# ponder-lab/RoaringBitmap

Hardware: AMD Instinct MI355X
Metric: input GB/s (HBM roofline %) for batched and/or/xor + wide-OR, 1/2/4/8 GPU (higher is better)
Workload: dtype u64

## Files before the change

### roaringbitmap_amd/csrc/pairwise.hip

```cpp
#include <algorithm>
#include "kernels.hpp"
#include "wave.hpp"

namespace rbg {

constexpr int kPairThreads = 256;

#ifndef RBG_SMALL_STUDY
#define RBG_SMALL_STUDY 0
#endif
#if RBG_SMALL_STUDY
constexpr int kStudyWords = 32;
__device__ uint64_t g_small_study[8192 * kStudyWords];
__device__ uint64_t g_merge_ts[8192 * 4][8];
#define RBG_MT(i) if (lane == 0) g_merge_ts[min(blockIdx.x, 8191u) * 4 + (threadIdx.x >> 6)][i] = __builtin_amdgcn_s_memrealtime()
#else
#define RBG_MT(i)
#endif

__device__ __forceinline__ bool keeps_a_only(int op) { return op != RB_AND; }
__device__ __forceinline__ bool keeps_b_only(int op) { return op == RB_OR || op == RB_XOR || is_lazy_op(op); }

__device__ __forceinline__ uint64_t alg_bytes(int t, uint32_t c, uint32_t r) {
  return t == kBitmap ? 8192ull : t == kArray ? 2ull * c : 4ull * r + 2;
// ... 855 lines not shown
  RecU cur = load_rec(recs + g);
  Task tc = decode_task<OP, ROLE == kRoleLight>(cur, pay_a, pay_b);
  uint4 pq[8], qq[8];
#if RBG_STUDY
  uint64_t lt_acc[8] = {0, 0, 0, 0, 0, 0, 0, 0}, lt0 = 0, lt1 = 0, lt2 = 0;
  uint64_t lt_wait = 0;
#define RBG_LT(x) if (ROLE == kRoleLight) { x; }
#define RBG_HT(x) if (ROLE == kRoleHeavy) { x; }
#else
#define RBG_LT(x)
#define RBG_HT(x)
#endif
  if (tc.kind == kCopy || tc.bigq) load_chunks(qq, tc.pp, 16, lane);
  else load_chunks(qq, tc.pq, tc.qbytes, lane);
  load_chunks(pq, tc.pp, tc.bigp ? 16u : tc.pbytes, lane);
  while (true) {
    uint64_t gn = g + stride;
    if (queue) {
      gn = g + 1;
      if (gn >= cend) {
        const Chunk c1 = claim_take(queue, n, qk, qtried, ticket, lane);
        gn = c1.s;
        cend = c1.e;
        if (qtried < kQueueStripes) ticket = claim_issue(queue, qk, lane);
      }
    }
    const bool has_next = gn < n;
    RBG_LT(lt0 = __builtin_amdgcn_s_memtime());
    RBG_HT(lt0 = __builtin_amdgcn_s_memtime());
    const RecU nx = load_rec(recs + (has_next ? gn : g));
    const Task tn = decode_task<OP, ROLE == kRoleLight>(nx, pay_a, pay_b);
    RBG_LT(lt1 = __builtin_amdgcn_s_memtime(); lt_acc[0] += lt1 - lt0);
    RBG_HT(lt1 = __builtin_amdgcn_s_memtime(); lt_acc[0] += lt1 - lt0);
    int ty = kEmpty, c = 0;
    uint32_t nr = 0, cw = 0xFFFFFFFFu;
    uint8_t *dst = out + cur.out;
    bool done = false;
    if (ROLE == kRoleHeavy && OP == RB_AND && tc.tp == kRun && tc.tq == kRun && !tc.bigp &&
        !tc.bigq && ((tc.rp + 3) & ~3u) + tc.rq <= 2048u) {
      int r = 0;
      done = and_runs_intervals<CARD_ONLY>(pq, qq, tc.rp, tc.rq, s, dst, lane, c, r);
      if (done) {
        ty = c == 0 ? kEmpty : CARD_ONLY ? kArray : kRun;
        nr = ty == kRun ? (uint32_t)r : 0u;
        __builtin_amdgcn_sched_barrier(0);
        {
          const bool real = has_next && !tn.bigq;
          load_chunks(qq, real ? tn.pq : tn.pp, real ? tn.qbytes : 16u, lane);
        }
        load_chunks(pq, tn.pp, tn.bigp ? 16u : tn.pbytes, lane);
      }
    }
    if (ROLE == kRoleHeavy && RBG_HEAVY_MERGE && !done && (OP == RB_OR || OP == RB_XOR) && !tm.lazy &&
        tc.tp == kArray && tc.tq == kArray && tc.cp + tc.cq <= kMergeMax) {
      merge_stage(pq, tc.cp, qq, tc.cq, s, lane);
      __builtin_amdgcn_sched_barrier(0);
      {
        const bool real = has_next && !tn.bigq;
        load_chunks(qq, real ? tn.pq : tn.pp, real ? tn.qbytes : 16u, lane);
      }
      load_chunks(pq, tn.pp, tn.bigp ? 16u : tn.pbytes, lane);
      c = (int)merge_run<OP, !CARD_ONLY>(s, tc.cp, tc.cq, reinterpret_cast<uint16_t *>(dst), lane);
      ty = CARD_ONLY ? (c ? kArray : kEmpty) : (c || (OP == RB_XOR && tm.keep_empty)) ? kArray : kEmpty;
      nr = 0;
      done = true;
    }
    if (ROLE == kRoleHeavy && !done) {
#if RBG_STUDY
      {
        const uint64_t tw0 = __builtin_amdgcn_s_memtime();
        __builtin_amdgcn_s_waitcnt(0x0F70);
        lt_wait += __builtin_amdgcn_s_memtime() - tw0;
      }
#endif
      uint64_t w[kW];
      if (bitmap_payload(tc.tp, tc.cp)) {
#pragma unroll
        for (int k = 0; k < 8; ++k) {
          w[2 * k] = pack2(pq[k].x, pq[k].y);
          w[2 * k + 1] = pack2(pq[k].z, pq[k].w);
        }
      } else if (tc.tp == kRun && !tc.bigp) {
        stage_run_toggles(pq, tc.rp, s, lane);
        lds_read_words(s, w, lane);
        wave_lds_sync();
        toggles_to_words(w, lane);
      } else {
        if (tc.bigp) stage_big_runs(tc.pp, tc.rp, s, lane);
        else stage_from_chunks(tc.tp, pq, tc.cp, tc.rp, s, lane);
        lds_read_words(s, w, lane);
        wave_lds_sync();
      }
      if (bitmap_payload(tc.tq, tc.cq)) {
#pragma unroll
        for (int k = 0; k < 8; ++k) {
          word_op<OP>(w[2 * k], pack2(qq[k].x, qq[k].y));
          word_op<OP>(w[2 * k + 1], pack2(qq[k].z, qq[k].w));
        }
      } else if (tc.tq == kRun && !tc.bigq) {
        stage_run_toggles(qq, tc.rq, s, lane);
        uint64_t t[kW];
        lds_read_words(s, t, lane);
        wave_lds_sync();
        toggles_to_words(t, lane);
#pragma unroll
        for (int j = 0; j < kW; ++j) word_op<OP>(w[j], t[j]);
      } else {
        if (tc.bigq) stage_big_runs(tc.pq, tc.rq, s, lane);
        else stage_from_chunks(tc.tq, qq, tc.cq, tc.rq, s, lane);
        const uint4 *s4 = reinterpret_cast<const uint4 *>(s);
#pragma unroll
        for (int k = 0; k < 8; ++k) {
          const uint4 v = s4[k * 64 + lane];
          word_op<OP>(w[2 * k], pack2(v.x, v.y));
          word_op<OP>(w[2 * k + 1], pack2(v.z, v.w));
        }
        wave_lds_sync();
      }
      RBG_HT(lt2 = __builtin_amdgcn_s_memtime(); lt_acc[1] += lt2 - lt1);
      __builtin_amdgcn_sched_barrier(0);
      {
        const bool real = has_next && !tn.bigq;
        load_chunks(qq, real ? tn.pq : tn.pp, real ? tn.qbytes : 16u, lane);
      }
      load_chunks(pq, tn.pp, tn.bigp ? 16u : tn.pbytes, lane);
      const int ta = tc.tp, tb = tc.tq;
      const bool lazy = OP == RB_OR && tm.lazy;
      const bool eff = eff_rule<OP>(ta, tb, tc.cp, tc.cq);
      int r;
      metrics(w, lane, (eff || (lazy && (ta == kRun || tb == kRun))) && !CARD_ONLY, c, r);
      RBG_HT(const uint64_t lt3 = __builtin_amdgcn_s_memtime(); lt_acc[2] += lt3 - lt2; lt2 = lt3);
      bool bits = false;
      if (lazy) {
        ty = lazy_or_type(tm.lazy, ta, tb, tc.cp, tc.cq, c, r, cw, bits);
        if (ty == kRun && c == kSpan) r = 1;
      } else if (OP != RB_OR && c == 0 && !(OP == RB_XOR && tm.keep_empty)) ty = kEmpty;
      else if (eff) ty = type_eff(c, r);
      else if (OP == RB_OR && tm.inplace && ta == kBitmap && tb == kArray) {
        ty = kBitmap;
      } else if (OP == RB_OR && (ta == kBitmap || tb == kBitmap)) {
        ty = type_lr(c);
        if (ty == kRun) r = 1;
      } else ty = type_ab(c);
      if (CARD_ONLY) ty = c ? kArray : kEmpty;
      else if (ty != kEmpty) {
        if (RBG_BAL_EMIT) emit_container_bal(bits ? (int)kBitmap : ty, w, c, r, dst, s, estage[wv], lane);
        else emit_container(bits ? (int)kBitmap : ty, w, c, r, dst, s, lane);
      }
      nr = ty == kRun ? (uint32_t)r : 0u;
      RBG_HT(lt_acc[3 + (ty == kBitmap ? 0 : ty == kArray ? 1 : 2)] += __builtin_amdgcn_s_memtime() - lt2);
    } else if (ROLE != kRoleHeavy) {
      if (tc.kind == kFilter || tc.kind == kBits) {
        if (tc.bigq) stage_big_runs(tc.pq, tc.rq, s, fresh(lane));
        else stage_from_chunks(tc.tq, qq, tc.cq, tc.rq, s, fresh(lane));
      } else if (!CARD_ONLY) {
        if (tc.bigp) {
          copy_payload(tc.pp, dst, tc.pbytes, fresh(lane), qq);
          __builtin_amdgcn_s_waitcnt(0x0F70);
        } else store_chunks(pq, dst, tc.pbytes, fresh(lane));
      }
      {
        const bool real = has_next && tn.kind != kCopy && !tn.bigq;
        load_chunks(qq, real ? tn.pq : tn.pp, real ? tn.qbytes : 16u, fresh(lane));
      }
      RBG_LT(lt2 = __builtin_amdgcn_s_memtime(); lt_acc[tc.kind == kFilter ? 1 + (tc.tq == kBitmap ? 0 : tc.tq == kArray ? 1 : 2) : 4] += lt2 - lt1);
      if (tc.kind == kFilter) {
        uint16_t *o = CARD_ONLY ? nullptr : reinterpret_cast<uint16_t *>(dst);
        uint4 *tb = tbuf[ROLE == kRoleLight ? wv : 0];
        c = OP == RB_ANDNOT ? filter_rows_linear<true, !CARD_ONLY>(pq, (int)tc.cp, s, ob, tb, o, fresh(lane))
                            : filter_rows_linear<false, !CARD_ONLY>(pq, (int)tc.cp, s, ob, tb, o, fresh(lane));
        ty = c ? kArray : kEmpty;
      } else if (tc.kind == kBits) {
        const uint4 *s4 = reinterpret_cast<const uint4 *>(s);
        uint32_t cl = 0;
#pragma unroll
        for (int k = 0; k < 8; ++k) {
          const uint4 x = s4[k * 64 + lane];
          pq[k] = make_uint4(pq[k].x | x.x, pq[k].y | x.y, pq[k].z | x.z, pq[k].w | x.w);
          cl += __popc(pq[k].x) + __popc(pq[k].y) + __popc(pq[k].z) + __popc(pq[k].w);
        }
        c = (int)wave_sum_u32(cl);
        const bool keep_bitmap = tm.inplace && tc.p_is_a && tc.tq == kArray;
        ty = c == kSpan && !keep_bitmap ? kRun : kBitmap;
        nr = ty == kRun ? 1u : 0u;
        if (!CARD_ONLY) {
          uint4 *o4 = reinterpret_cast<uint4 *>(dst);
          if (ty == kRun) {
            if (lane == 0) o4[0] = make_uint4(0xFFFF0000u, 0u, 0u, 0u);
          } else {
#pragma unroll
            for (int k = 0; k < 8; ++k) o4[k * 64 + lane] = pq[k];
          }
        }
        if (CARD_ONLY) {
          ty = kArray;
          nr = 0;
        }
      } else {
        ty = tc.tp;
        c = (int)tc.cp;
        nr = tc.rp;
      }
      RBG_LT(lt_acc[5] += __builtin_amdgcn_s_memtime() - lt2);
      load_chunks(pq, tn.pp, tn.bigp ? 16u : tn.pbytes, fresh(lane));
    }
    wave_lds_sync();
    if (lane == 0) {
      tm.type[cur.t] = (uint8_t)ty;
      tm.res[cur.t] = task_res((uint32_t)ty, nr, cw != 0xFFFFFFFFu ? cw : (uint32_t)c);
    }
    RBG_LT(lt_acc[6] += __builtin_amdgcn_s_memtime() - lt0; ++lt_acc[7]);
    RBG_HT(lt_acc[6] += __builtin_amdgcn_s_memtime() - lt0; ++lt_acc[7]);
    if (!has_next) break;
    g = gn;
    cur = nx;
    tc = tn;
  }
#if RBG_STUDY
  if (ROLE == kRoleLight && lane == 0 && wv == 0 && blockIdx.x % 97 == 0)
    printf("light timing blk %u: decode %lu stageB %lu stageA %lu stageR %lu copy %lu filter %lu iter %lu tasks %lu\n",
           blockIdx.x, lt_acc[0], lt_acc[1], lt_acc[2], lt_acc[3], lt_acc[4], lt_acc[5], lt_acc[6], lt_acc[7]);
  if (ROLE == kRoleHeavy && lane == 0 && wv == 0 && blockIdx.x % 61 == 0)
    printf("heavy timing op %d blk %u: decode %lu build %lu (payload wait %lu) metrics %lu emitB %lu emitA %lu emitR %lu iter %lu tasks %lu\n",
           OP, blockIdx.x, lt_acc[0], lt_acc[1], lt_wait, lt_acc[2], lt_acc[3], lt_acc[4], lt_acc[5], lt_acc[6], lt_acc[7]);
#endif
}

__device__ __forceinline__ uint32_t fold_chunks(const uint4 (&q)[8]) {
  uint32_t x = 0;
#pragma unroll
  for (int i = 0; i < 8; ++i) x ^= q[i].x ^ q[i].y ^ q[i].z ^ q[i].w;
  return x;
}
template <int OP>
__global__ __launch_bounds__(256, 4) void k_probe_tasks(const uint8_t *__restrict__ pay_a,
                                                     const uint8_t *__restrict__ pay_b,
                                                     const TaskRec *__restrict__ recs, uint64_t n, uint32_t *sink) {
  const int lane = lane_id();
  const int wv = __builtin_amdgcn_readfirstlane(threadIdx.x >> 6);
  const uint64_t stride = (uint64_t)gridDim.x * 4;
  uint64_t g = (uint64_t)blockIdx.x * 4 + wv;
  if (g >= n) return;
  RecU cur = load_rec(recs + g);
  Task tc = decode_task<OP, false>(cur, pay_a, pay_b);
  uint4 pq[8], qq[8];
  load_chunks(pq, tc.pp, tc.bigp ? 16u : tc.pbytes, lane);
  if (tc.kind == kCopy || tc.bigq) load_chunks(qq, tc.pp, 16, lane);
  else load_chunks(qq, tc.pq, tc.qbytes, lane);
  uint32_t acc = 0;
  while (true) {
    const uint64_t gn = g + stride;
    const bool has_next = gn < n;
    const RecU nx = load_rec(recs + (has_next ? gn : g));
    const Task tn = decode_task<OP, false>(nx, pay_a, pay_b);
    acc ^= fold_chunks(qq);
    {
      const bool real = has_next && tn.kind != kCopy && !tn.bigq;
      load_chunks(qq, real ? tn.pq : tn.pp, real ? tn.qbytes : 16u, lane);
    }
    acc ^= fold_chunks(pq);
    load_chunks(pq, tn.pp, tn.bigp ? 16u : tn.pbytes, lane);
    if (!has_next) break;
    g = gn;
    tc = tn;
  }
  sink[(uint64_t)blockIdx.x * 256 + threadIdx.x] = acc;
}
__global__ __launch_bounds__(256, 4) void k_probe_stream(const uint8_t *__restrict__ p, uint64_t bytes,
                                                      uint32_t *sink) {
  const int lane = lane_id();
  const uint64_t w = (uint64_t)blockIdx.x * 4 + (threadIdx.x >> 6), nw = (uint64_t)gridDim.x * 4;
  const uint64_t chunks = bytes / 8192;
  uint32_t acc = 0;
  for (uint64_t c = w; c < chunks; c += nw) {
    uint4 q[8];
    load_chunks(q, p + c * 8192, 8192, lane);
    acc ^= fold_chunks(q);
  }
  sink[(uint64_t)blockIdx.x * 256 + threadIdx.x] = acc;
}
void launch_probe(int op, int mode, const uint8_t *pa, const uint8_t *pb, uint64_t a_bytes, const TaskRec *recs,
                  uint64_t n, uint32_t *sink, unsigned blocks, hipStream_t st) {
  if (mode == 2) {
    k_probe_stream<<<blocks, 256, 0, st>>>(pa, a_bytes, sink);
    return;
  }
  if (!n) return;
  switch (op) {
  case RB_AND: k_probe_tasks<RB_AND><<<blocks, 256, 0, st>>>(pa, pb, recs, n, sink); break;
  case RB_OR: k_probe_tasks<RB_OR><<<blocks, 256, 0, st>>>(pa, pb, recs, n, sink); break;
  case RB_XOR: k_probe_tasks<RB_XOR><<<blocks, 256, 0, st>>>(pa, pb, recs, n, sink); break;
  default: k_probe_tasks<RB_ANDNOT><<<blocks, 256, 0, st>>>(pa, pb, recs, n, sink); break;
  }
}

__global__ __launch_bounds__(kPairThreads) void k_compact_count(const uint64_t *tb, uint64_t nseg,
                                                                const uint8_t *ttype, uint64_t *bk) {
  const uint64_t p = (uint64_t)blockIdx.x * kPairThreads + threadIdx.x;
  uint64_t n = 0;
  if (p < nseg)
    for (uint64_t t = tb[p]; t < tb[p + 1]; ++t) n += ttype[t] != kEmpty;
  const uint64_t v[1] = {n};
  uint64_t sum[1];
  block_sums(v, sum);
  if (threadIdx.x == 0) bk[blockIdx.x] = sum[0];
}
__global__ __launch_bounds__(kPairThreads) void k_compact_write(const uint64_t *tb, uint64_t nseg, TaskMeta tm,
                                                                const uint64_t *bks, OutView out,
                                                                const uint32_t *seg_pair, uint64_t *pair_card,
                                                                uint64_t *stats, uint64_t *rseg, uint64_t *rbegin,
                                                                CallTail tail) {
  __shared__ uint32_t wtot[kPairThreads / 64];
  const uint64_t b0 = (uint64_t)blockIdx.x * kPairThreads, be = min(b0 + kPairThreads, nseg);
  const uint64_t p = b0 + threadIdx.x;
  const uint64_t R0 = bks[blockIdx.x];
  uint32_t kept = 0;
  const uint64_t t0 = p < nseg ? tb[p] : 0, t1 = p < nseg ? tb[p + 1] : 0;
  for (uint64_t t = t0; t < t1; ++t) kept += tm.type[t] != kEmpty;
  uint32_t btot;
  const uint64_t rs = R0 + block_xscan(kept, wtot, btot);
  if (p < nseg) {
    if (rseg) rseg[p] = rs;
    if (rbegin) rbegin[p] = rs;
// ... 752 lines not shown
```

### roaringbitmap_amd/csrc/wave.hpp

```cpp
#pragma once
#include "common.hpp"

namespace rbg {

constexpr int kW = 16;

__device__ __forceinline__ void wave_lds_sync() {
  __builtin_amdgcn_fence(__ATOMIC_RELEASE, "wavefront");
  __builtin_amdgcn_wave_barrier();
  __builtin_amdgcn_fence(__ATOMIC_ACQUIRE, "wavefront");
}

__device__ __forceinline__ int lane_id() { return (int)(threadIdx.x & 63); }
__device__ __forceinline__ int fresh(int x) {
  asm volatile("" : "+v"(x));
  return x;
}

__device__ __forceinline__ uint32_t xcd_swizzle(uint32_t orig, uint32_t nwg) {
  const uint32_t q = nwg / 8, r = nwg % 8, xcd = orig % 8;
  return (xcd < r ? xcd * (q + 1) : r * (q + 1) + (xcd - r) * q) + orig / 8;
}

template <int CTRL, int ROW_MASK = 0xf, bool BOUND_ZERO = true>
__device__ __forceinline__ uint32_t dpp(uint32_t x) {
  return (uint32_t)__builtin_amdgcn_update_dpp(0, (int)x, CTRL, ROW_MASK, 0xf, BOUND_ZERO);
}
__device__ __forceinline__ uint32_t readlane(uint32_t x, int l) {
  return (uint32_t)__builtin_amdgcn_readlane((int)x, l);
}
__device__ __forceinline__ uint32_t wave_scan_u32(uint32_t v, int ) {
  v += dpp<0x111>(v);
  v += dpp<0x112>(v);
  v += dpp<0x114>(v);
  v += dpp<0x118>(v);
  v += dpp<0x142, 0xa, false>(v);
  v += dpp<0x143, 0xc, false>(v);
  return v;
}
__device__ __forceinline__ uint32_t wave_xscan_xor(uint32_t v, int ) {
  v ^= dpp<0x111>(v);
  v ^= dpp<0x112>(v);
  v ^= dpp<0x114>(v);
  v ^= dpp<0x118>(v);
  v ^= dpp<0x142, 0xa, false>(v);
  v ^= dpp<0x143, 0xc, false>(v);
  return v;
}
__device__ __forceinline__ uint64_t wave_scan_u64(uint64_t v, int lane) {
  return (uint64_t)wave_scan_u32((uint32_t)v, lane) | ((uint64_t)wave_scan_u32((uint32_t)(v >> 32), lane) << 32);
}
__device__ __forceinline__ uint32_t wave_sum_u32(uint32_t v) { return readlane(wave_scan_u32(v, 0), 63); }
__device__ __forceinline__ uint64_t wave_sum_u64(uint64_t v) {
#pragma unroll
  for (int o = 32; o > 0; o >>= 1) v += (uint64_t)__shfl_xor((unsigned long long)v, o);
  return v;
}
__device__ __forceinline__ uint32_t wave_max_u32(uint32_t v) {
#pragma unroll
  for (int o = 32; o > 0; o >>= 1) v = max(v, (uint32_t)__shfl_xor((int)v, o));
  return v;
}

__device__ __forceinline__ uint64_t pack2(uint32_t lo, uint32_t hi) { return (uint64_t)lo | ((uint64_t)hi << 32); }

__device__ __forceinline__ void load_bitmap(const uint8_t *p, uint64_t (&w)[kW], int lane) {
  const uint4 *q = reinterpret_cast<const uint4 *>(p);
  uint4 v[8];
#pragma unroll
  for (int k = 0; k < 8; ++k) v[k] = q[k * 64 + lane];
#pragma unroll
  for (int k = 0; k < 8; ++k) {
    w[2 * k] = pack2(v[k].x, v[k].y);
    w[2 * k + 1] = pack2(v[k].z, v[k].w);
  }
}
__device__ __forceinline__ void lds_zero(uint32_t *s, int lane) {
  uint4 *s4 = reinterpret_cast<uint4 *>(s);
#pragma unroll
  for (int k = 0; k < 8; ++k) s4[k * 64 + lane] = make_uint4(0, 0, 0, 0);
}
__device__ __forceinline__ void lds_read_words(const uint32_t *s, uint64_t (&w)[kW], int lane) {
  const uint4 *s4 = reinterpret_cast<const uint4 *>(s);
#pragma unroll
  for (int k = 0; k < 8; ++k) {
    uint4 v = s4[k * 64 + lane];
    w[2 * k] = pack2(v.x, v.y);
    w[2 * k + 1] = pack2(v.z, v.w);
  }
}

__device__ __forceinline__ void lds_write_words(uint32_t *s, const uint64_t (&w)[kW], int lane) {
  uint4 *s4 = reinterpret_cast<uint4 *>(s);
#pragma unroll
  for (int k = 0; k < 8; ++k)
    s4[k * 64 + lane] = make_uint4((uint32_t)w[2 * k], (uint32_t)(w[2 * k] >> 32), (uint32_t)w[2 * k + 1],
                                   (uint32_t)(w[2 * k + 1] >> 32));
}

template <bool XOR = false>
__device__ __forceinline__ void or_chunk_values(const uint32_t (&x)[8], int n, uint32_t *s) {
  uint32_t acc = 0, prev = x[0] >> 5;
  const uint32_t lastw = x[n - 1 < 7 ? n - 1 : 7] >> 5;
#pragma unroll
  for (int i = 0; i < 8; ++i) {
    const bool live = i < n;
    const uint32_t wi = live ? x[i] >> 5 : lastw;
    acc = (wi == prev ? acc : 0u) | (live ? 1u << (x[i] & 31) : 0u);
    prev = wi;
    const bool last = (!XOR || live) && (i == 7 || i + 1 >= n || (x[i + 1] >> 5) != wi);
    if (XOR) atomicXor(&s[wi], last ? acc : 0u);
    else atomicOr(&s[wi], last ? acc : 0u);
  }
}

__device__ __forceinline__ void lds_or_array(const uint16_t *vals, int card, uint32_t *s, int lane) {
  const uint4 *v4 = reinterpret_cast<const uint4 *>(vals);
  const int nchunks = (card + 7) >> 3;
  for (int c = lane; c < nchunks; c += 64) {
    uint4 q = v4[c];
    uint32_t x[8] = {q.x & 0xFFFF, q.x >> 16, q.y & 0xFFFF, q.y >> 16,
                     q.z & 0xFFFF, q.z >> 16, q.w & 0xFFFF, q.w >> 16};
    or_chunk_values(x, min(8, card - 8 * c), s);
  }
}

__device__ __forceinline__ void expand_array(const uint16_t *vals, int card, uint32_t *s,
                                             uint64_t (&w)[kW], int lane) {
  lds_zero(s, lane);
  wave_lds_sync();
  lds_or_array(vals, card, s, lane);
  wave_lds_sync();
  lds_read_words(s, w, lane);
  wave_lds_sync();
}

__device__ __forceinline__ uint64_t prefix_xor64(uint64_t x) {
  x ^= x << 1;
  x ^= x << 2;
  x ^= x << 4;
  x ^= x << 8;
  x ^= x << 16;
  x ^= x << 32;
  return x;
}

__device__ __forceinline__ void toggles_to_words(uint64_t (&t)[kW], int lane) {
  uint32_t q = 0, p0 = 0;
#pragma unroll
  for (int k = 0; k < 8; ++k) {
    uint32_t a = __popcll(t[2 * k]) & 1, b = __popcll(t[2 * k + 1]) & 1;
    q |= (a ^ b) << k;
    p0 |= a << k;
  }
  const uint32_t incl = wave_xscan_xor(q, lane);
  const uint32_t excl = incl ^ q;
  const uint32_t tot = readlane(incl, 63);
#pragma unroll
  for (int k = 0; k < 8; ++k) {
    uint32_t rowc = __popc(tot & ((1u << k) - 1)) & 1;
    uint32_t c0 = rowc ^ ((excl >> k) & 1);
    uint32_t c1 = c0 ^ ((p0 >> k) & 1);
    t[2 * k] = prefix_xor64(t[2 * k]) ^ (c0 ? ~0ull : 0ull);
    t[2 * k + 1] = prefix_xor64(t[2 * k + 1]) ^ (c1 ? ~0ull : 0ull);
  }
}

__device__ __forceinline__ void toggles_to_words_lds(uint32_t *s, int lane) {
  uint4 *s4 = reinterpret_cast<uint4 *>(s);
  uint32_t q = 0, p0 = 0;
#pragma unroll
  for (int k = 0; k < 8; ++k) {
    const uint4 v = s4[k * 64 + lane];
    const uint32_t a = (__popc(v.x) + __popc(v.y)) & 1, b = (__popc(v.z) + __popc(v.w)) & 1;
    q |= (a ^ b) << k;
    p0 |= a << k;
  }
  const uint32_t incl = wave_xscan_xor(q, lane);
  const uint32_t excl = incl ^ q;
  const uint32_t tot = readlane(incl, 63);
#pragma unroll
  for (int k = 0; k < 8; ++k) {
    const uint4 v = s4[k * 64 + lane];
    const uint32_t rowc = __popc(tot & ((1u << k) - 1)) & 1;
    const uint32_t c0 = rowc ^ ((excl >> k) & 1);
    const uint32_t c1 = c0 ^ ((p0 >> k) & 1);
    const uint64_t w0 = prefix_xor64(pack2(v.x, v.y)) ^ (c0 ? ~0ull : 0ull);
    const uint64_t w1 = prefix_xor64(pack2(v.z, v.w)) ^ (c1 ? ~0ull : 0ull);
    s4[k * 64 + lane] = make_uint4((uint32_t)w0, (uint32_t)(w0 >> 32), (uint32_t)w1, (uint32_t)(w1 >> 32));
    __builtin_amdgcn_sched_barrier(0);
  }
}

__device__ __forceinline__ void toggle_run(uint32_t *s, uint32_t q) {
  const uint32_t st = q & 0xFFFF, e1 = st + (q >> 16) + 1;
  atomicXor(&s[st >> 5], 1u << (st & 31));
  if (e1 < (uint32_t)kSpan) atomicXor(&s[e1 >> 5], 1u << (e1 & 31));
}

__device__ __forceinline__ void expand_runs(const uint16_t *runs, int nruns, uint32_t *s,
                                            uint64_t (&w)[kW], int lane) {
  lds_zero(s, lane);
  wave_lds_sync();
  const uint32_t *r32 = reinterpret_cast<const uint32_t *>(runs);
  for (int i = lane; i < nruns; i += 64) toggle_run(s, r32[i]);
  wave_lds_sync();
  lds_read_words(s, w, lane);
  wave_lds_sync();
  toggles_to_words(w, lane);
}

__device__ __forceinline__ void load_container(int type, const uint8_t *p, uint32_t card, uint32_t nruns,
                                               uint32_t *s, uint64_t (&w)[kW], int lane) {
  if (type == kBitmap) load_bitmap(p, w, lane);
  else if (type == kArray) expand_array(reinterpret_cast<const uint16_t *>(p), (int)card, s, w, lane);
  else expand_runs(reinterpret_cast<const uint16_t *>(p), (int)nruns, s, w, lane);
}

__device__ __forceinline__ void stage_container(int type, const uint8_t *p, uint32_t card, uint32_t nruns,
                                                uint32_t *s, int lane) {
  if (type == kBitmap) {
    const uint4 *q = reinterpret_cast<const uint4 *>(p);
    uint4 v[8];
#pragma unroll
    for (int k = 0; k < 8; ++k) v[k] = q[k * 64 + lane];
    uint4 *s4 = reinterpret_cast<uint4 *>(s);
#pragma unroll
    for (int k = 0; k < 8; ++k) s4[k * 64 + lane] = v[k];
  } else if (type == kArray) {
    lds_zero(s, lane);
    wave_lds_sync();
    lds_or_array(reinterpret_cast<const uint16_t *>(p), (int)card, s, lane);
  } else {
    uint64_t w[kW];
    expand_runs(reinterpret_cast<const uint16_t *>(p), (int)nruns, s, w, lane);
    lds_write_words(s, w, lane);
  }
  wave_lds_sync();
}

__device__ __forceinline__ uint32_t block_xscan(uint32_t v, uint32_t *wtot, uint32_t &total) {
  const int lane = lane_id(), w = threadIdx.x >> 6, nw = blockDim.x >> 6;
  const uint32_t inc = wave_scan_u32(v, lane);
  if (lane == 63) wtot[w] = inc;
  __syncthreads();
  uint32_t before = 0;
  total = 0;
  for (int i = 0; i < nw; ++i) {
    const uint32_t t = wtot[i];
    if (i < w) before += t;
    total += t;
  }
  __syncthreads();
  return before + inc - v;
}
#if defined(__HIP_DEVICE_COMPILE__) && !defined(__gfx950__) && !defined(__gfx942__)
#error "the one-launch hand-off (st_sc1 / ld_sc1 + s_waitcnt vmcnt) is written for gfx942 / gfx950"
#endif
__device__ __forceinline__ void st_sc1(uint64_t *p, uint64_t v) {
  __hip_atomic_store(p, v, __ATOMIC_RELAXED, __HIP_MEMORY_SCOPE_AGENT);
}
__device__ __forceinline__ uint64_t ld_sc1(const uint64_t *p) {
  return __hip_atomic_load(const_cast<uint64_t *>(p), __ATOMIC_RELAXED, __HIP_MEMORY_SCOPE_AGENT);
}

__device__ __forceinline__ __amdgpu_buffer_rsrc_t chunk_rsrc(const uint8_t *p, uint32_t bytes) {
  return __builtin_amdgcn_make_buffer_rsrc(const_cast<uint8_t *>(p), (short)0, (int)((bytes + 15) & ~15u), 0x00020000);
}
__device__ __forceinline__ uint4 load_chunk_row(__amdgpu_buffer_rsrc_t rs, int i, int lane) {
  typedef unsigned int v4u __attribute__((ext_vector_type(4)));
  const v4u v = __builtin_amdgcn_raw_buffer_load_b128(rs, (lane + 64 * i) * 16, 0, 0);
  return make_uint4(v.x, v.y, v.z, v.w);
}
__device__ __forceinline__ void load_chunks(uint4 (&q)[8], const uint8_t *p, uint32_t bytes, int lane) {
  const __amdgpu_buffer_rsrc_t rs = chunk_rsrc(p, bytes);
#pragma unroll
  for (int i = 0; i < 8; ++i) q[i] = load_chunk_row(rs, i, lane);
}
__device__ __forceinline__ uint32_t mbcnt64(uint64_t m) {
  return __builtin_amdgcn_mbcnt_hi((uint32_t)(m >> 32), __builtin_amdgcn_mbcnt_lo((uint32_t)m, 0u));
}
__device__ __forceinline__ uint32_t block_flag_count(bool f, uint32_t *wt) {
  const uint64_t m = __ballot(f);
  if ((threadIdx.x & 63) == 0) wt[threadIdx.x >> 6] = (uint32_t)__popcll(m);
  __syncthreads();
  return wt[0] + wt[1] + wt[2] + wt[3];
}
__device__ __forceinline__ uint32_t block_flag_rank(bool f, uint32_t *wt) {
  const uint64_t m = __ballot(f);
  const int w = threadIdx.x >> 6;
  if ((threadIdx.x & 63) == 0) wt[w] = (uint32_t)__popcll(m);
  __syncthreads();
  uint32_t r = mbcnt64(m);
  for (int i = 0; i < w; ++i) r += wt[i];
  return r;
}
constexpr int kStageRing = 576;
constexpr int kStageVals = kStageRing + 64;
template <bool NEGATE, bool STORE>
__device__ __forceinline__ int filter_rows_linear(const uint4 (&fq)[8], int nf, const uint32_t *s, uint16_t *ob,
                                                  uint4 *tb, uint16_t *out, int lane) {
  static_assert(7 + 512 <= kStageRing, "every slot (pending < 8, + < 512 of a row) lies below the dummies");
  const int iters = (nf + 511) >> 9;
  uint32_t tot = 0, flushed = 0;
  uint4 *out4 = reinterpret_cast<uint4 *>(out);
  uint4 *ob4 = reinterpret_cast<uint4 *>(ob);
  const uint16_t *t16 = reinterpret_cast<const uint16_t *>(tb);
  typedef __attribute__((address_space(3))) const uint32_t lds_u32;
  lds_u32 *ls = (lds_u32 *)s;
#pragma unroll
  for (int i = 0; i < 8; ++i) {
    if (i < iters) {
#pragma unroll
      for (int hf = 0; hf < 2; ++hf) {
        if (hf == 1 && nf - 512 * i <= 256) continue;
        if ((lane >> 5) == hf) tb[lane & 31] = fq[i];
        wave_lds_sync();
        const int nh = min(256, nf - 512 * i - 256 * hf);
        uint32_t y[4], m[4];
#pragma unroll
        for (int k = 0; k < 4; ++k) y[k] = t16[64 * k + lane];
#pragma unroll
        for (int k = 0; k < 4; ++k) {
          uint32_t wi;
          asm("v_bfe_u32 %0, %1, 5, 11" : "=v"(wi) : "v"(y[k]));
          m[k] = ls[wi];
        }
#pragma unroll
        for (int k = 0; k < 4; ++k) {
          const uint32_t bit = __builtin_amdgcn_ubfe(m[k], y[k], 1u);
          uint64_t b = __builtin_amdgcn_uicmp(bit, 0u, NEGATE ? 32 : 33);
          const int lim = nh - 64 * k;
          if (lim < 64) b &= lim > 0 ? (1ull << lim) - 1ull : 0ull;
          if (STORE) {
            const uint32_t pos =
                __builtin_amdgcn_mbcnt_hi((uint32_t)(b >> 32), __builtin_amdgcn_mbcnt_lo((uint32_t)b, tot - flushed));
            uint32_t slot;
            asm("v_cndmask_b32 %0, %1, %2, %3" : "=v"(slot) : "v"((uint32_t)(kStageRing + lane)), "v"(pos), "s"(b));
            ob[slot] = (uint16_t)y[k];
          }
          tot += (uint32_t)__popcll(b);
        }
      }
      if (STORE) {
        wave_lds_sync();
        const uint32_t pend = tot - flushed, nb = pend >> 3;
        if ((uint32_t)lane < nb) out4[(flushed >> 3) + lane] = ob4[lane];
        if (lane == 0 && nb && (pend & 7u)) ob4[0] = ob4[nb];
        wave_lds_sync();
        flushed += nb << 3;
      }
    }
    __builtin_amdgcn_sched_barrier(0);
  }
  if (STORE && tot > flushed && lane == 0) out4[flushed >> 3] = ob4[0];
  return (int)tot;
}

__device__ __forceinline__ void store_chunks(const uint4 (&q)[8], uint8_t *p, uint32_t bytes, int lane) {
  uint4 *p4 = reinterpret_cast<uint4 *>(p);
  const int n = (int)((bytes + 15) >> 4);
#pragma unroll
  for (int i = 0; i < 8; ++i) {
    const int c = lane + 64 * i;
    if (c < n) p4[c] = q[i];
  }
}

__device__ __forceinline__ void stage_run_toggles(const uint4 (&q)[8], uint32_t nruns, uint32_t *s, int lane) {
  lds_zero(s, lane);
  wave_lds_sync();
  const int nchunks = (int)((nruns + 3) >> 2);
#pragma unroll
  for (int i = 0; i < 8; ++i) {
    const int c = lane + 64 * i;
    if (c < nchunks) {
      const uint32_t r[4] = {q[i].x, q[i].y, q[i].z, q[i].w};
      uint32_t x[8];
#pragma unroll
      for (int k = 0; k < 4; ++k) {
        x[2 * k] = r[k] & 0xFFFF;
        x[2 * k + 1] = (r[k] & 0xFFFF) + (r[k] >> 16) + 1;
      }
      const int nr = min(4, (int)nruns - 4 * c);
      int n = 2 * nr;
      const uint32_t last = nr == 4 ? x[7] : nr == 3 ? x[5] : nr == 2 ? x[3] : x[1];
      if (last >= (uint32_t)kSpan) --n;
      or_chunk_values(x, n, s);
    }
  }
  wave_lds_sync();
}

__device__ __forceinline__ void stage_from_chunks(int type, const uint4 (&q)[8], uint32_t card, uint32_t nruns,
                                                  uint32_t *s, int lane) {
  uint4 *s4 = reinterpret_cast<uint4 *>(s);
  if (type == kBitmap) {
#pragma unroll
    for (int i = 0; i < 8; ++i) s4[i * 64 + lane] = q[i];
  } else {
    lds_zero(s, lane);
    wave_lds_sync();
    if (type == kArray) {
      const int nchunks = (int)((card + 7) >> 3);
#pragma unroll
      for (int i = 0; i < 8; ++i) {
        const int c = lane + 64 * i;
        if (c < nchunks) {
          const uint32_t x[8] = {q[i].x & 0xFFFF, q[i].x >> 16, q[i].y & 0xFFFF, q[i].y >> 16,
                                 q[i].z & 0xFFFF, q[i].z >> 16, q[i].w & 0xFFFF, q[i].w >> 16};
          or_chunk_values(x, min(8, (int)card - 8 * c), s);
        }
      }
    } else {
      const int nchunks = (int)((nruns + 3) >> 2);
#pragma unroll
      for (int i = 0; i < 8; ++i) {
        const int c = lane + 64 * i;
        if (c < nchunks) {
          const uint32_t r[4] = {q[i].x, q[i].y, q[i].z, q[i].w};
          uint32_t x[8];
#pragma unroll
          for (int k = 0; k < 4; ++k) {
            x[2 * k] = r[k] & 0xFFFF;
            x[2 * k + 1] = (r[k] & 0xFFFF) + (r[k] >> 16) + 1;
          }
          const int nr = min(4, (int)nruns - 4 * c);
          int n = 2 * nr;
          const uint32_t last = nr == 4 ? x[7] : nr == 3 ? x[5] : nr == 2 ? x[3] : x[1];
          if (last >= (uint32_t)kSpan) --n;
          or_chunk_values(x, n, s);
        }
      }
      wave_lds_sync();
      toggles_to_words_lds(s, lane);
    }
  }
  wave_lds_sync();
}

struct Neigh {
  uint32_t prev_top_h0;
  uint32_t next_bot_h1;
};
__device__ __forceinline__ Neigh neighbours(const uint64_t (&w)[kW], int lane) {
  uint32_t top1 = 0, bot0 = 0;
#pragma unroll
  for (int k = 0; k < 8; ++k) {
    top1 |= (uint32_t)(w[2 * k + 1] >> 63) << k;
    bot0 |= (uint32_t)(w[2 * k] & 1) << k;
  }
  const uint32_t up = dpp<0x138>(top1);
  const uint32_t last = readlane(top1, 63);
  const uint32_t dn = dpp<0x130>(bot0);
  const uint32_t first = readlane(bot0, 0);
  Neigh n;
  n.prev_top_h0 = lane ? up : ((last << 1) & 0xFE);
  n.next_bot_h1 = lane < 63 ? dn : ((first >> 1) & 0x7F);
  return n;
}
__device__ __forceinline__ uint64_t run_starts(const uint64_t (&w)[kW], const Neigh &n, int j) {
  const int k = j >> 1;
  uint64_t prev = (j & 1) ? (w[j - 1] >> 63) : (uint64_t)((n.prev_top_h0 >> k) & 1);
  return w[j] & ~((w[j] << 1) | prev);
}
__device__ __forceinline__ uint64_t run_ends(const uint64_t (&w)[kW], const Neigh &n, int j) {
  const int k = j >> 1;
  uint64_t next = (j & 1) ? (uint64_t)((n.next_bot_h1 >> k) & 1) : (w[j + 1] & 1);
  return w[j] & ~((w[j] >> 1) | (next << 63));
}
__device__ __forceinline__ uint32_t lane_card(const uint64_t (&w)[kW]) {
  uint32_t c = 0;
#pragma unroll
  for (int j = 0; j < kW; ++j) c += __popcll(w[j]);
  return c;
}
__device__ __forceinline__ void metrics(const uint64_t (&w)[kW], int lane, bool want_runs, int &card,
                                        int &runs) {
  uint32_t c = lane_card(w);
  uint32_t r = 0;
  if (want_runs) {
    Neigh n = neighbours(w, lane);
#pragma unroll
    for (int j = 0; j < kW; ++j) r += __popcll(run_starts(w, n, j));
  }
  card = (int)wave_sum_u32(c);
  runs = want_runs ? (int)wave_sum_u32(r) : 0;
}

__device__ __forceinline__ int type_ab(int c) { return c <= kMaxArray ? kArray : kBitmap; }
__device__ __forceinline__ int type_eff(int c, int r) {
  return 2 + 4 * r <= min(kBitmapBytes, 2 * c + 2) ? kRun : type_ab(c);
}
__device__ __forceinline__ int type_lr(int c) {
  return c <= kMaxArray ? kArray : (c == kSpan ? kRun : kBitmap);
}
__device__ __forceinline__ int type_runopt(int c, int r) {
  if (c <= kMaxArray) return 2 * c > 2 + 4 * r ? kRun : kArray;
  return kBitmapBytes > 2 + 4 * r ? kRun : kBitmap;
}

__device__ __forceinline__ uint32_t emit_container(int type, const uint64_t (&w)[kW], int card, int runs,
                                                   uint8_t *out, uint32_t *s, int lane) {
  if (type == kBitmap) {
    uint4 *o = reinterpret_cast<uint4 *>(out);
#pragma unroll
    for (int k = 0; k < 8; ++k)
      o[k * 64 + lane] = make_uint4((uint32_t)w[2 * k], (uint32_t)(w[2 * k] >> 32),
                                    (uint32_t)w[2 * k + 1], (uint32_t)(w[2 * k + 1] >> 32));
    return kBitmapBytes;
  }
  uint16_t *s16 = reinterpret_cast<uint16_t *>(s);
  if (type == kArray) {
    uint32_t n[8];
#pragma unroll
    for (int k = 0; k < 8; ++k) n[k] = __popcll(w[2 * k]) + __popcll(w[2 * k + 1]);
    const uint64_t P0 = (uint64_t)n[0] | ((uint64_t)n[1] << 16) | ((uint64_t)n[2] << 32) | ((uint64_t)n[3] << 48);
    const uint64_t P1 = (uint64_t)n[4] | ((uint64_t)n[5] << 16) | ((uint64_t)n[6] << 32) | ((uint64_t)n[7] << 48);
    const uint64_t S0 = wave_scan_u64(P0, lane), S1 = wave_scan_u64(P1, lane);
    const uint64_t E0 = S0 - P0, E1 = S1 - P1;
    const uint64_t T0 = pack2(readlane((uint32_t)S0, 63), readlane((uint32_t)(S0 >> 32), 63));
    const uint64_t T1 = pack2(readlane((uint32_t)S1, 63), readlane((uint32_t)(S1 >> 32), 63));
    uint32_t rowoff = 0;
#pragma unroll
    for (int k = 0; k < 8; ++k) {
      const uint64_t E = k < 4 ? E0 : E1, T = k < 4 ? T0 : T1;
      const int sh = 16 * (k & 3);
      uint32_t pos = rowoff + (uint32_t)((E >> sh) & 0xFFFF);
      rowoff += (uint32_t)((T >> sh) & 0xFFFF);
#pragma unroll
      for (int h = 0; h < 2; ++h) {
        uint64_t x = w[2 * k + h];
        const uint32_t base = (uint32_t)(128 * k + 2 * lane + h) << 6;
        while (x) {
          s16[pos++] = (uint16_t)(base + __builtin_ctzll(x));
          x &= x - 1;
        }
      }
    }
    wave_lds_sync();
    const uint32_t bytes = 2u * (uint32_t)card;
    const uint4 *s4 = reinterpret_cast<const uint4 *>(s);
    uint4 *o = reinterpret_cast<uint4 *>(out);
    for (uint32_t i = lane; i * 16 < bytes; i += 64) o[i] = s4[i];
    wave_lds_sync();
    return bytes;
  }
  Neigh nb = neighbours(w, lane);
  uint32_t ns[8];
#pragma unroll
  for (int k = 0; k < 8; ++k) ns[k] = __popcll(run_starts(w, nb, 2 * k)) + __popcll(run_starts(w, nb, 2 * k + 1));
  const uint64_t P0 = (uint64_t)ns[0] | ((uint64_t)ns[1] << 16) | ((uint64_t)ns[2] << 32) | ((uint64_t)ns[3] << 48);
  const uint64_t P1 = (uint64_t)ns[4] | ((uint64_t)ns[5] << 16) | ((uint64_t)ns[6] << 32) | ((uint64_t)ns[7] << 48);
  const uint64_t S0 = wave_scan_u64(P0, lane), S1 = wave_scan_u64(P1, lane);
  const uint64_t E0 = S0 - P0, E1 = S1 - P1;
  const uint64_t T0 = pack2(readlane((uint32_t)S0, 63), readlane((uint32_t)(S0 >> 32), 63));
  const uint64_t T1 = pack2(readlane((uint32_t)S1, 63), readlane((uint32_t)(S1 >> 32), 63));
  uint16_t *S = s16, *E = s16 + 2048;
  uint32_t rowoff = 0;
#pragma unroll
  for (int k = 0; k < 8; ++k) {
    const uint64_t Ex = k < 4 ? E0 : E1, T = k < 4 ? T0 : T1;
    const int sh = 16 * (k & 3);
    uint32_t sp = rowoff + (uint32_t)((Ex >> sh) & 0xFFFF);
    rowoff += (uint32_t)((T >> sh) & 0xFFFF);
#pragma unroll
    for (int h = 0; h < 2; ++h) {
      const int j = 2 * k + h;
      const uint32_t open = (uint32_t)(h ? (w[j - 1] >> 63) : ((nb.prev_top_h0 >> k) & 1)) & (uint32_t)(w[j] & 1);
      uint32_t ep = sp - open;
      const uint32_t base = (uint32_t)(128 * k + 2 * lane + h) << 6;
      uint64_t x = run_starts(w, nb, j), y = run_ends(w, nb, j);
      while (x | y) {
        if (x) {
          S[sp++] = (uint16_t)(base + __builtin_ctzll(x));
          x &= x - 1;
        }
        if (y) {
          E[ep++] = (uint16_t)(base + __builtin_ctzll(y));
          y &= y - 1;
        }
      }
    }
  }
  wave_lds_sync();
  const uint2 *S2 = reinterpret_cast<const uint2 *>(S), *E2 = reinterpret_cast<const uint2 *>(E);
  uint4 *o4 = reinterpret_cast<uint4 *>(out);
  for (int i = lane; 4 * i < runs; i += 64) {
// ... 141 lines not shown
```

Before: 3743.

## Skip full prefix-xor for run filters; probe toggles by parity; simplify LDS atomics

```diff
diff --git a/roaringbitmap_amd/csrc/pairwise.hip b/roaringbitmap_amd/csrc/pairwise.hip
--- a/roaringbitmap_amd/csrc/pairwise.hip
+++ b/roaringbitmap_amd/csrc/pairwise.hip
@@ -1031,7 +1031,7 @@
     } else if (ROLE != kRoleHeavy) {
       if (tc.kind == kFilter || tc.kind == kBits) {
         if (tc.bigq) stage_big_runs(tc.pq, tc.rq, s, fresh(lane));
-        else stage_from_chunks(tc.tq, qq, tc.cq, tc.rq, s, fresh(lane));
+        else stage_from_chunks(tc.tq, qq, tc.cq, tc.rq, s, fresh(lane), tc.kind == kFilter);
       } else if (!CARD_ONLY) {
         if (tc.bigp) {
           copy_payload(tc.pp, dst, tc.pbytes, fresh(lane), qq);
@@ -1046,8 +1046,10 @@
       if (tc.kind == kFilter) {
         uint16_t *o = CARD_ONLY ? nullptr : reinterpret_cast<uint16_t *>(dst);
         uint4 *tb = tbuf[ROLE == kRoleLight ? wv : 0];
-        c = OP == RB_ANDNOT ? filter_rows_linear<true, !CARD_ONLY>(pq, (int)tc.cp, s, ob, tb, o, fresh(lane))
-                            : filter_rows_linear<false, !CARD_ONLY>(pq, (int)tc.cp, s, ob, tb, o, fresh(lane));
+        constexpr bool kNeg = OP == RB_ANDNOT;
+        if (tc.tq == kRun && !tc.bigq)
+          c = filter_rows_linear<kNeg, !CARD_ONLY, true>(pq, (int)tc.cp, s, ob, tb, o, fresh(lane));
+        else c = filter_rows_linear<kNeg, !CARD_ONLY, false>(pq, (int)tc.cp, s, ob, tb, o, fresh(lane));
         ty = c ? kArray : kEmpty;
       } else if (tc.kind == kBits) {
         const uint4 *s4 = reinterpret_cast<const uint4 *>(s);
diff --git a/roaringbitmap_amd/csrc/wave.hpp b/roaringbitmap_amd/csrc/wave.hpp
--- a/roaringbitmap_amd/csrc/wave.hpp
+++ b/roaringbitmap_amd/csrc/wave.hpp
@@ -100,17 +100,16 @@
 
 template <bool XOR = false>
 __device__ __forceinline__ void or_chunk_values(const uint32_t (&x)[8], int n, uint32_t *s) {
-  uint32_t acc = 0, prev = x[0] >> 5;
-  const uint32_t lastw = x[n - 1 < 7 ? n - 1 : 7] >> 5;
+  typedef __attribute__((address_space(3))) uint32_t lds_u32;
+  lds_u32 *ls = (lds_u32 *)s;
+  const uint32_t live = (1u << n) - 1u;
 #pragma unroll
   for (int i = 0; i < 8; ++i) {
-    const bool live = i < n;
-    const uint32_t wi = live ? x[i] >> 5 : lastw;
-    acc = (wi == prev ? acc : 0u) | (live ? 1u << (x[i] & 31) : 0u);
-    prev = wi;
-    const bool last = (!XOR || live) && (i == 7 || i + 1 >= n || (x[i + 1] >> 5) != wi);
-    if (XOR) atomicXor(&s[wi], last ? acc : 0u);
-    else atomicOr(&s[wi], last ? acc : 0u);
+    uint32_t wi;
+    asm("v_bfe_u32 %0, %1, 5, 11" : "=v"(wi) : "v"(x[i]));
+    const uint32_t bit = __builtin_amdgcn_ubfe(live, (uint32_t)i, 1u) << (x[i] & 31);
+    if (XOR) __hip_atomic_fetch_xor(ls + wi, bit, __ATOMIC_RELAXED, __HIP_MEMORY_SCOPE_WORKGROUP);
+    else __hip_atomic_fetch_or(ls + wi, bit, __ATOMIC_RELAXED, __HIP_MEMORY_SCOPE_WORKGROUP);
   }
 }
 
@@ -188,6 +187,30 @@
     const uint64_t w0 = prefix_xor64(pack2(v.x, v.y)) ^ (c0 ? ~0ull : 0ull);
     const uint64_t w1 = prefix_xor64(pack2(v.z, v.w)) ^ (c1 ? ~0ull : 0ull);
     s4[k * 64 + lane] = make_uint4((uint32_t)w0, (uint32_t)(w0 >> 32), (uint32_t)w1, (uint32_t)(w1 >> 32));
+    __builtin_amdgcn_sched_barrier(0);
+  }
+}
+
+__device__ __forceinline__ void toggles_fold_carry_lds(uint32_t *s, int lane) {
+  uint4 *s4 = reinterpret_cast<uint4 *>(s);
+  uint32_t q = 0;
+#pragma unroll
+  for (int k = 0; k < 8; ++k) {
+    const uint4 v = s4[k * 64 + lane];
+    q |= ((__popc(v.x) + __popc(v.y) + __popc(v.z) + __popc(v.w)) & 1u) << k;
+  }
+  const uint32_t incl = wave_xscan_xor(q, lane);
+  const uint32_t excl = incl ^ q;
+  const uint32_t tot = readlane(incl, 63);
+#pragma unroll
+  for (int k = 0; k < 8; ++k) {
+    uint4 v = s4[k * 64 + lane];
+    const uint32_t rowc = __popc(tot & ((1u << k) - 1)) & 1;
+    v.x ^= rowc ^ ((excl >> k) & 1);
+    v.y ^= __popc(v.x) & 1;
+    v.z ^= __popc(v.y) & 1;
+    v.w ^= __popc(v.z) & 1;
+    s4[k * 64 + lane] = v;
     __builtin_amdgcn_sched_barrier(0);
   }
 }
@@ -297,7 +320,7 @@
 }
 constexpr int kStageRing = 576;
 constexpr int kStageVals = kStageRing + 64;
-template <bool NEGATE, bool STORE>
+template <bool NEGATE, bool STORE, bool PARITY = false>
 __device__ __forceinline__ int filter_rows_linear(const uint4 (&fq)[8], int nf, const uint32_t *s, uint16_t *ob,
                                                   uint4 *tb, uint16_t *out, int lane) {
   static_assert(7 + 512 <= kStageRing, "every slot (pending < 8, + < 512 of a row) lies below the dummies");
@@ -328,7 +351,7 @@
         }
 #pragma unroll
         for (int k = 0; k < 4; ++k) {
-          const uint32_t bit = __builtin_amdgcn_ubfe(m[k], y[k], 1u);
+          const uint32_t bit = PARITY ? (uint32_t)__popc(m[k] << (~y[k] & 31u)) & 1u : __builtin_amdgcn_ubfe(m[k], y[k], 1u);
           uint64_t b = __builtin_amdgcn_uicmp(bit, 0u, NEGATE ? 32 : 33);
           const int lim = nh - 64 * k;
           if (lim < 64) b &= lim > 0 ? (1ull << lim) - 1ull : 0ull;
@@ -393,7 +416,7 @@
 }
 
 __device__ __forceinline__ void stage_from_chunks(int type, const uint4 (&q)[8], uint32_t card, uint32_t nruns,
-                                                  uint32_t *s, int lane) {
+                                                  uint32_t *s, int lane, bool fold_runs = false) {
   uint4 *s4 = reinterpret_cast<uint4 *>(s);
   if (type == kBitmap) {
 #pragma unroll
@@ -433,7 +456,8 @@
         }
       }
       wave_lds_sync();
-      toggles_to_words_lds(s, lane);
+      if (fold_runs) toggles_fold_carry_lds(s, lane);
+      else toggles_to_words_lds(s, lane);
     }
   }
   wave_lds_sync();
```

New measurement: 3950, median of 6. 1.06x the previous value.
